# robustrobotics/multi_view_stereonet

Hardware: AMD Instinct MI355X
Metric: depthmaps/sec at 512x256, 64 hypotheses, 2 src views; L1 vs ref (higher is better)
Workload: dtype f32; 1 GPU; GTA-SfM-shaped 512x256, D=64 hypotheses, 2 source views, cost-volume filter + 5 refiners; global_batch=256, parallelism=dp1 (independent images, all-gather of metric rows)

## Files before the change

multi_view_stereonet_amd/csrc/mvsn_conv_wino.hip:

```cpp
#include <type_traits>
#include <utility>

#include "mvsn_resident.h"
#include "mvsn_conv_wino.h"

namespace mvsn {

constexpr int WN_THREADS = 512, WN_WAVES = 8;
constexpr int WN_TY = 16, WN_TX = 32;
constexpr int WN_WIDE_TY = 10, WN_WIDE_TX = 40, WN_WIDE_PC = WN_WIDE_TX / 2, WN_WIDE_NP = (WN_WIDE_TY / 2) * WN_WIDE_PC;
constexpr int WN_ROLL_PR = 6, WN_ROLL_NP = WN_ROLL_PR * WN_WIDE_PC, WN_ROLL_HY = 2 * WN_ROLL_PR + 3;
constexpr int WN_TILE_RP = 3;
constexpr int wn_pa(int dil) { return (dil + 3) / 4 * 4; }
constexpr int WN_UFLOATS = 16 * 128;
constexpr int WN_MAX_CHUNKS = 9;
constexpr int WN_LDS_MAX = 160 * 1024;

__device__ floatx4 g_wn_zero16 = {0.f, 0.f, 0.f, 0.f};

#ifndef MVSN_WN_ABLATE
#define MVSN_WN_ABLATE 0
#endif

#ifndef MVSN_RD_ABLATE
// ... 796 lines not shown
#pragma unroll
      for (int rr = 0; rr < 2; ++rr) {
        const bool rok = rr ? row1 : row0;
#pragma unroll
        for (int h = 0; h < 2; ++h) {
          const bool ok = rok && (h ? q1 : q0);
          if (rok && (!(MVSN_WN_ABLATE & 64) || n < 0))
            wn_store4<MVSN_WN_NT_STORES ? 2 : 0>(
                osrd, h ? ovoff1 : ovoff0, (unsigned)(((size_t)(t * 16) * cstride + (size_t)rr * DIL * g.W) * 4),
                floatx4{y[t][rr][4 * h], y[t][rr][4 * h + 1], y[t][rr][4 * h + 2], y[t][rr][4 * h + 3]});
          if (ok) {
#pragma unroll
            for (int k = 0; k < 4; ++k) s[t] += y[t][rr][4 * h + k];
          }
        }
      }
    }
    WN_STAMP();
    if (out_partials != nullptr) {
      auto sum8 = [](float v) {
        v += dpp_mov<0xB1>(v);
        v += dpp_mov<0x4E>(v);
        v += dpp_mov<0x141>(v);
        return v;
      };
      const int hi = (lq >> 3) & 1;
      const float npos = 8.0f * (float)cnt;
      const float rn = cnt == 16 ? 0.0078125f : (cnt == 8 ? 0.015625f : (cnt == 4 ? 0.03125f : 0.0f));
      float m[2], qv[2] = {0.f, 0.f};
#pragma unroll
      for (int t = 0; t < 2; ++t) {
        s[t] = sum8(s[t]);
        m[t] = s[t] * rn;
      }
#pragma unroll
      for (int t = 0; t < 2; ++t)
#pragma unroll
        for (int rr = 0; rr < 2; ++rr)
#pragma unroll
          for (int h = 0; h < 2; ++h)
            if ((rr ? row1 : row0) && (h ? q1 : q0)) {
#pragma unroll
              for (int k = 0; k < 4; ++k) {
                const float dv = y[t][rr][4 * h + k] - m[t];
                qv[t] += dv * dv;
              }
            }
#pragma unroll
      for (int t = 0; t < 2; ++t) qv[t] = sum8(qv[t]);
      int rtile = tile_id, rwave = wave;
      bool rec_ok = true;
      if constexpr (RP) {
        const int yq = oy & (TY - 1);
        rtile = (oy / TY) * g.ntx + x0 / TX, rwave = yq / (2 * DIL) * DIL + yq % DIL;
        rec_ok = oy < g.nty * TY;
      }
      if ((lq & 7) == 0 && rec_ok) {
        float *rec = out_partials + (((size_t)n * (RP ? g.tiles : ptiles) + (size_t)z * g.tiles + rtile) * WN_WAVES + rwave) * 48;
        rec += gq * 12 + hi * 3;
#pragma unroll
        for (int t = 0; t < 2; ++t) {
          rec[t * 6 + 0] = npos;
          rec[t * 6 + 1] = m[t];
          rec[t * 6 + 2] = qv[t];
        }
      }
    }
  };

  auto finish_tile_tr = [&](int n, int z, int tile_id, int y0, int x0, int r_s) {
    int lq;
    asm volatile("v_mbcnt_lo_u32_b32 %0, -1, 0\n\tv_mbcnt_hi_u32_b32 %0, -1, %0" : "=v"(lq));
    const int pc = lq & 15, gq = lq >> 4;
    int oy = y0 + 2 * wave, ox = x0 + 2 * pc;
    bool slot_ok = true;
    unsigned zb = 0;
    if constexpr (WIDE != 0) {
      const int q = wave * 16 + pc;
      slot_ok = q < NP;
      const int qq = slot_ok ? q : 0, pr = qq / WN_WIDE_PC;
      oy = y0 + 2 * pr, ox = x0 + 2 * (qq - pr * WN_WIDE_PC);
      if constexpr (ROLL) {
        const bool pb = pr >= r_s;
        oy = pb ? 2 * (pr - r_s) : oy;
        zb = pb ? (unsigned)plane : 0u;
        slot_ok = slot_ok & (!pb | (z + 1 < g.D));
      }
    }
    const bool row0 = oy < g.H, row1 = oy + 1 < g.H, cok = slot_ok && ox < g.W;
    const size_t cstride = VOL ? (size_t)g.D * plane : plane;
    const __amdgpu_buffer_rsrc_t osrd = wn_rsrc(out + (size_t)n * 32 * cstride + (size_t)z * plane, (unsigned)(32 * cstride * 4));
    const unsigned ovoff = cok ? ((unsigned)(4 * gq) * (unsigned)cstride + zb + (unsigned)(oy * g.W + ox)) * 4u : 0xFFFFFFFFu;
    const unsigned ovoff0 = (!WIDE || row0) ? ovoff : 0xFFFFFFFFu, ovoff1 = (!WIDE || row1) ? ovoff : 0xFFFFFFFFu;
    float s[2] = {0.f, 0.f};
    float y[2][4][4];
#pragma unroll
    for (int t = 0; t < 2; ++t) {
      const floatx4 bv = *reinterpret_cast<const floatx4 *>(bias_lds + t * 16 + 4 * gq);
#pragma unroll
      for (int r = 0; r < 4; ++r) {
        float s0[4], s1[4];
#pragma unroll
        for (int j = 0; j < 4; ++j) {
          s0[j] = acc[j][t][r] + acc[4 + j][t][r] + acc[8 + j][t][r];
          s1[j] = acc[4 + j][t][r] - acc[8 + j][t][r] - acc[12 + j][t][r];
        }
        y[t][r][0] = s0[0] + s0[1] + s0[2] + bv[r];
        y[t][r][1] = s0[1] - s0[2] - s0[3] + bv[r];
        y[t][r][2] = s1[0] + s1[1] + s1[2] + bv[r];
        y[t][r][3] = s1[1] - s1[2] - s1[3] + bv[r];
        if (!(MVSN_WN_ABLATE & 64) || n < 0) {
          const unsigned so = (unsigned)((size_t)(t * 16 + r) * cstride * 4);
          if (WIDE || row0) wn_store2<MVSN_WN_NT_TR ? 2 : 0>(osrd, ovoff0, so, y[t][r][0], y[t][r][1]);
          if (WIDE || row1) wn_store2<MVSN_WN_NT_TR ? 2 : 0>(osrd, ovoff1, so + (unsigned)g.W * 4u, y[t][r][2], y[t][r][3]);
        }
        if (row0 && cok) s[t] += y[t][r][0] + y[t][r][1];
        if (row1 && cok) s[t] += y[t][r][2] + y[t][r][3];
      }
    }
    WN_STAMP();
    if (out_partials != nullptr) {
      auto sum16 = [](float v) {
        v += dpp_mov<0xB1>(v);
        v += dpp_mov<0x4E>(v);
        v += dpp_mov<0x141>(v);
        v += dpp_mov<0x140>(v);
        return v;
      };
      const int vp = (g.W - x0) >> 1;
      float npos = (float)(8 * ((row0 ? 1 : 0) + (row1 ? 1 : 0)) * (vp > 16 ? 16 : vp));
      if constexpr (WIDE != 0)
        npos = sum16(cok ? (float)(8 * ((row0 ? 1 : 0) + (row1 ? 1 : 0))) : 0.0f);
      float m[2], qv[2] = {0.f, 0.f};
#pragma unroll
      for (int t = 0; t < 2; ++t) {
        s[t] = sum16(s[t]);
        m[t] = npos > 0.f ? s[t] / npos : 0.f;
      }
#pragma unroll
      for (int t = 0; t < 2; ++t)
#pragma unroll
        for (int r = 0; r < 4; ++r)
#pragma unroll
          for (int k = 0; k < 4; ++k)
            if ((k < 2 ? row0 : row1) && cok) {
              const float dv = y[t][r][k] - m[t];
              qv[t] += dv * dv;
            }
#pragma unroll
      for (int t = 0; t < 2; ++t) qv[t] = sum16(qv[t]);
      if (pc < 4) {
        float *rec = out_partials + (((size_t)n * ptiles + (ROLL ? (size_t)0 : (size_t)z * g.tiles) + tile_id) * WN_WAVES + wave) * 48;
        rec += gq * 12 + pc * 3;
        const int ga = gq >> 1;
        const bool a = pc == ga, b = pc == 2 + ga;
        rec[0] = (a || b) ? npos : 0.f;
        rec[1] = a ? m[0] : (b ? m[1] : 0.f);
        rec[2] = a ? qv[0] : (b ? qv[1] : 0.f);
      }
    }
  };

  int step = 0, mm_stage = 0;
  for (int round = 0; round < my_items; ++round) {
#ifdef MVSN_WN_STAMPS
    dbg_on = round >= 3 || my_items < 4;
#endif
    const int flat = g.rev ? total - 1 - (round * G + slot) : round * G + slot;
    const int n = flat / ptiles;
    int tile_id = flat - n * ptiles, z = 0;
    int r_pr0 = 0, r_s = WN_ROLL_PR;
    if constexpr (ROLL) {
      roll_item(tile_id, z, r_pr0, r_s);
    } else if constexpr (VOL) {
      z = tile_id / g.tiles;
      tile_id -= z * g.tiles;
    }
    const int tyi = ROLL ? 0 : wdiv(tile_id, g.fd_ntx), txi = ROLL ? 0 : tile_id - tyi * g.ntx;
    const int y0 = ROLL ? 2 * r_pr0 : item_y0(tyi), x0 = txi * TX;

#pragma unroll
    for (int xi = 0; xi < 16; ++xi) asm volatile("" : "=v"(acc[xi][0]), "=v"(acc[xi][1]));

    int chunk = 0;
    auto do_step = [&](auto firstc) {
      const bool has_next = step + 1 < total_steps;
      bool waited = false;
      if constexpr (RIDE > 0) {
        if constexpr (ASM_RIDE) {
          if (rd_young != PERV) asm volatile("s_waitcnt vmcnt(0)" ::: "memory");
          asm volatile("s_waitcnt vmcnt(%0)" ::"n"(PERV) : "memory");
        } else if (rd_young == PERV) asm volatile("s_waitcnt vmcnt(%0)" ::"n"(PERV) : "memory");
        else if (rd_young == PER) asm volatile("s_waitcnt vmcnt(%0)" ::"n"(PER) : "memory");
        else if (VOL && rd_young == 2) asm volatile("s_waitcnt vmcnt(2)" ::: "memory");
        else asm volatile("s_waitcnt vmcnt(0)" ::: "memory");
        rd_consume(lane);
        waited = true;
      }
      if (has_next) {
        const int rest = total_steps - (step + 2);
        if (!waited) wait_landed(rest < 0 ? 0 : (rest < NSTAGE - 2 ? rest : NSTAGE - 2));
        xf_apply();
        WN_STAMP();
        if (!(MVSN_WN_ABLATE & 8)) wn_barrier<LDS_BARRIER>();
        if (MVSN_WN_STAGGER > 0 && wave >= 4) __builtin_amdgcn_s_sleep(MVSN_WN_STAGGER);
        WN_STAMP();
        xf_prepare();
      }
      rd_issue(flat, chunk);
      float dn[KS][4][4];
      if (has_next && !(MVSN_WN_ABLATE & 32)) {
        if (MVSN_WN_XF == 1) tr_load(dn);
        else if (MVSN_WN_XF == 0) tr_load(dn, 0, 1);
      }
      auto multiply = [&](auto first, auto hc) {
        constexpr bool FIRST = decltype(first)::value;
        constexpr int h = decltype(hc)::value;
        const float *ub = U + (VOL ? mm_stage : chunk) * UST + h * WN_UFLOATS + lane;
        float fb[2][2];
        fb[0][0] = ub[0], fb[0][1] = ub[64];
        auto tcol = [&](int i, int j) {
          const float d0 = dn[h][0][dslot(j)], d1 = dn[h][1][dslot(j)], d2 = dn[h][2][dslot(j)], d3 = dn[h][3][dslot(j)];
          return i == 0 ? d0 - d2 : (i == 1 ? d1 + d2 : (i == 2 ? d2 - d1 : d1 - d3));
        };
        constexpr bool INTER = MVSN_WN_XF == 1 || (MVSN_WN_XF == 0 && h == 0);
        float tc[4], tn[4];
        if constexpr (INTER) {
#pragma unroll
          for (int j = 0; j < 4; ++j) tc[j] = tcol(0, j);
        } else {
          if (has_next && !(MVSN_WN_ABLATE & 32)) tr_load(dn, h, h + 1);
        }
#pragma unroll
        for (int xi = 0; xi < 16; ++xi) {
          const int cur = xi & 1, ti = xi >> 2, tj = xi & 3;
          if (INTER && ti < 3) tn[tj] = tcol(ti + 1, tj);
          if (xi + 1 < 16 && !(MVSN_WN_ABLATE & 2)) {
            fb[cur ^ 1][0] = ub[(xi + 1) * 128];
            fb[cur ^ 1][1] = ub[(xi + 1) * 128 + 64];
          }
          if constexpr (FIRST) {
            acc[xi][0] = TR ? mfma16x16x4(fb[cur][0], v[h][xi], floatx4{0.f, 0.f, 0.f, 0.f})
                            : mfma16x16x4(v[h][xi], fb[cur][0], floatx4{0.f, 0.f, 0.f, 0.f});
            acc[xi][1] = TR ? mfma16x16x4(fb[cur][1], v[h][xi], floatx4{0.f, 0.f, 0.f, 0.f})
                            : mfma16x16x4(v[h][xi], fb[cur][1], floatx4{0.f, 0.f, 0.f, 0.f});
          } else {
            acc[xi][0] = TR ? mfma16x16x4(fb[cur][0], v[h][xi], acc[xi][0]) : mfma16x16x4(v[h][xi], fb[cur][0], acc[xi][0]);
            acc[xi][1] = TR ? mfma16x16x4(fb[cur][1], v[h][xi], acc[xi][1]) : mfma16x16x4(v[h][xi], fb[cur][1], acc[xi][1]);
          }
          if (h == 0 && xi == 1 && has_next && !(MVSN_WN_ABLATE & 4)) {
            pf_issue();
            uq_issue();
          }
          if constexpr (INTER) {
            if (!(MVSN_WN_ABLATE & 1)) {
              v[h][xi] = tj == 0 ? tc[0] - tc[2] : (tj == 1 ? tc[1] + tc[2] : (tj == 2 ? tc[2] - tc[1] : tc[1] - tc[3]));
              if (MVSN_WN_PIN) asm volatile("" : "+v"(v[h][xi]));
            }
            if (tj == 3) {
#pragma unroll
              for (int k = 0; k < 4; ++k) tc[k] = tn[k];
            }
          }
          __builtin_amdgcn_sched_barrier(0);
        }
        if constexpr (!INTER) {
          if (!(MVSN_WN_ABLATE & 1)) {
            tr_finish(dn, v, h, h + 1);
#pragma unroll
            for (int xi = 0; xi < 16; ++xi)
              if (MVSN_WN_PIN) asm volatile("" : "+v"(v[h][xi]));
          }
          __builtin_amdgcn_sched_barrier(0);
        }
      };
      multiply(firstc, std::integral_constant<int, 0>{});
      if constexpr (KS == 2) multiply(std::false_type{}, std::integral_constant<int, 1>{});
      tr_advance();
      if constexpr (VOL) mm_stage = mm_stage + 1 == NSTAGE ? 0 : mm_stage + 1;
      WN_STAMP();
      ++step;
    };
    do_step(std::true_type{});
    for (chunk = 1; chunk < nsteps; ++chunk) do_step(std::false_type{});
    if (!(MVSN_WN_ABLATE & 16) || n < 0) {
      if constexpr (TR) finish_tile_tr(n, z, tile_id, y0, x0, r_s);
      else finish_tile(n, z, tile_id, y0, x0);
    }
  }
  if constexpr (RIDE > 0) {
    if (total_steps > 0) {
      asm volatile("s_waitcnt vmcnt(0)" ::: "memory");
      int ln;
      asm volatile("v_mbcnt_lo_u32_b32 %0, -1, 0\n\tv_mbcnt_hi_u32_b32 %0, -1, %0" : "=v"(ln));
      rd_consume(ln);
    }
  }
#ifdef MVSN_WN_STAMPS
  if (dbg)
    for (int i = 0; i < dbg_i; ++i) dbg[i] = dbg_lds[i];
#endif
}

constexpr int S2_TY = 16, S2_TX = 32;
constexpr int S2_ROWS = 2 * S2_TY + 3, S2_XS = 2 * S2_TX + 8, S2_DQ = S2_XS / 4;
constexpr int S2_GROUPS = S2_ROWS * S2_DQ, S2_PIECES = (S2_GROUPS + 63) / 64;
constexpr int S2_RCST = S2_ROWS * S2_XS + 1;
constexpr int S2_STAGE = 4 * S2_RCST;
constexpr int S2_UST = 4 * WN_UFLOATS;
constexpr int S2_STEPS = 8;
constexpr size_t S2_LDS_BYTES = (size_t)(2 * S2_STAGE + 2 * S2_UST + 32) * sizeof(float);
static_assert(S2_PIECES * 4 % WN_WAVES == 0, "a step's raw pieces divide evenly among the waves");
static_assert(S2_LDS_BYTES <= 160 * 1024, "LDS plan");

__global__ void wino_s2_pack_kernel(const float *__restrict__ w, float *__restrict__ out) {
  const int idx = blockIdx.x * blockDim.x + threadIdx.x;
  if (idx >= S2_STEPS * S2_UST) return;
  const int lane = idx & 63, t = (idx >> 6) & 1, xi = (idx >> 7) & 15, ph = (idx >> 11) & 3, cc = idx >> 13;
  const int py = ph >> 1, px = ph & 1;
  const int co = t * 16 + (lane & 15), ci = cc * 4 + (lane >> 4);
  const float *g = w + ((size_t)co * 32 + ci) * 25;
  const float G[4][3] = {{1.f, 0.f, 0.f}, {0.5f, 0.5f, 0.5f}, {0.5f, -0.5f, 0.5f}, {0.f, 0.f, 1.f}};
  const int i = xi >> 2, j = xi & 3;
  float u = 0.0f;
  for (int a = 0; a < 3; ++a)
    for (int b = 0; b < 3; ++b) {
      const int ky = 2 * a + py, kx = 2 * b + px;
      if (ky < 5 && kx < 5) u += G[i][a] * g[ky * 5 + kx] * G[j][b];
    }
  out[idx] = u;
}

#ifndef MVSN_S2_PIN
#define MVSN_S2_PIN 1
#endif
#ifndef MVSN_S2_CNTWAIT
#define MVSN_S2_CNTWAIT 1
#endif
struct WinoS2Args {
  int n, H, W, Ho, Wo, ntx, tiles;
  WinoDiv fd_ntx;
};

__global__ __launch_bounds__(WN_THREADS, 2) void conv_wino_s2_kernel(WinoS2Args g, const float *__restrict__ in,
                                                                     const float *__restrict__ upk,
                                                                     const float *__restrict__ bias,
                                                                     float *__restrict__ out) {
  extern __shared__ __attribute__((aligned(16))) float smem[];
  float *U = smem + 2 * S2_STAGE;
  float *bias_lds = U + 2 * S2_UST;
  const int tid = threadIdx.x, lane = tid & 63;
  const int wave = __builtin_amdgcn_readfirstlane(tid >> 6);
  const size_t plane = (size_t)g.H * g.W;
  const int oplane = g.Ho * g.Wo;
  const int total = g.n * g.tiles, G = gridDim.x;
  const int slot = xcd_tile_index(blockIdx.x, G);
  const int my_items = slot < total ? (total - slot + G - 1) / G : 0;
  const int total_steps = my_items * S2_STEPS;
  if (tid < 32) bias_lds[tid] = bias ? bias[tid] : 0.0f;

  constexpr int PER = S2_PIECES * 4 / WN_WAVES;
  const int dch = wave >> 1, dp0 = (wave & 1) * PER;
  int pf_item = 0, pf_cc = 0, pf_n = 0;
  int pf_goff[PER];
  auto pf_plan = [&]() {
    const int flat = pf_item * G + slot;
    const int n = flat / g.tiles, tile = flat - n * g.tiles;
    const int tyi = wdiv(tile, g.fd_ntx), txi = tile - tyi * g.ntx;
    const int gy0 = 2 * tyi * S2_TY - 2, gx0 = 2 * txi * S2_TX - 4;
    pf_n = n;
    int lo;
    asm volatile("v_mbcnt_lo_u32_b32 %0, -1, 0\n\tv_mbcnt_hi_u32_b32 %0, -1, %0" : "=v"(lo));
#pragma unroll
    for (int i = 0; i < PER; ++i) {
      const int e = (dp0 + i) * 64 + lo;
      const int row = e / S2_DQ, q = e - row * S2_DQ;
      const int gy = gy0 + row, gx = gx0 + 4 * q;
      pf_goff[i] = (gy >= 0 && gy < g.H && gx >= 0 && gx < g.W) ? (gy * g.W + gx) * 4 : -1;
    }
  };
  auto pf_issue = [&](int step) {
    if (step >= total_steps) return;
    const float *src = in + ((size_t)pf_n * 32 + pf_cc * 4 + dch) * plane;
    float *dst = smem + (step & 1) * S2_STAGE + dch * S2_RCST;
#pragma unroll
    for (int i = 0; i < PER; ++i)
      if ((dp0 + i) * 64 + lane < S2_GROUPS)
        wn_dma16_buf<true>(src, (unsigned)plane * 4u, (unsigned)pf_goff[i], dst + (dp0 + i) * 256);
    const float *us = upk + (size_t)pf_cc * S2_UST + wave * 1024 + lane * 4;
    float *ud = U + (step & 1) * S2_UST + wave * 1024;
#pragma unroll
    for (int i = 0; i < 4; ++i) wn_dma16<true>(us + i * 256, ud + i * 256);
    if (++pf_cc == S2_STEPS) {
      pf_cc = 0;
      ++pf_item;
      if (pf_item < my_items) pf_plan();
    }
  };
  if (my_items > 0) pf_plan();
  pf_issue(0);

  const int pcol = lane & 15, kc = lane >> 4;
  const int rbase = kc * S2_RCST + (4 * wave) * S2_XS + 4 * pcol + 2;

  floatx4 acc[16][2];
#pragma unroll
  for (int xi = 0; xi < 16; ++xi) acc[xi][0] = acc[xi][1] = floatx4{0.f, 0.f, 0.f, 0.f};

  int item = 0, cc = 0;
  for (int step = 0; step < total_steps; ++step) {
    if (MVSN_S2_CNTWAIT && cc == 0 && step > 0) asm volatile("s_waitcnt vmcnt(8)" ::: "memory");
    else asm volatile("s_waitcnt vmcnt(0)" ::: "memory");
    wn_barrier<true>();
    pf_issue(step + 1);
    const float *raw = smem + (step & 1) * S2_STAGE + rbase;
    const float *us = U + (step & 1) * S2_UST + lane;
#pragma unroll
    for (int py = 0; py < 2; ++py) {
      typedef float s2_f2 __attribute__((ext_vector_type(2)));
      s2_f2 d[4][4];
#pragma unroll
      for (int i = 0; i < 4; ++i)
#pragma unroll
        for (int j = 0; j < 4; ++j) {
          const float *q = raw + (py + 2 * i) * S2_XS + 2 * j;
          d[i][j] = (py && i == 3) ? s2_f2{0.f, 0.f} : s2_f2{q[0], q[1]};
        }
      s2_f2 t[4][4], v[16];
#pragma unroll
      for (int j = 0; j < 4; ++j) {
        t[0][j] = d[0][j] - d[2][j];
        t[1][j] = d[1][j] + d[2][j];
        t[2][j] = d[2][j] - d[1][j];
        t[3][j] = d[1][j] - d[3][j];
      }
#pragma unroll
      for (int i = 0; i < 4; ++i) {
        v[i * 4 + 0] = t[i][0] - t[i][2];
        v[i * 4 + 1] = t[i][1] + t[i][2];
        v[i * 4 + 2] = t[i][2] - t[i][1];
        v[i * 4 + 3] = t[i][1] - t[i][3];
      }
      if (MVSN_S2_PIN) {
#pragma unroll
        for (int xi = 0; xi < 16; ++xi)
          if (!(py && (xi >> 2) == 3)) asm volatile("" : "+v"(v[xi]));
      }
#pragma unroll
      for (int xi = 0; xi < 16; ++xi) {
        if (py && (xi >> 2) == 3) continue;
        const float *u = us + ((py * 2) * 16 + xi) * 128;
        acc[xi][0] = mfma16x16x4(v[xi].x, u[0], acc[xi][0]);
        acc[xi][1] = mfma16x16x4(v[xi].x, u[64], acc[xi][1]);
        if ((xi & 3) != 3) {
          acc[xi][0] = mfma16x16x4(v[xi].y, u[16 * 128], acc[xi][0]);
          acc[xi][1] = mfma16x16x4(v[xi].y, u[16 * 128 + 64], acc[xi][1]);
        }
      }
    }
    if (++cc == S2_STEPS) {
      cc = 0;
      const int flat = item * G + slot;
      const int n = flat / g.tiles, tile = flat - n * g.tiles;
      const int tyi = wdiv(tile, g.fd_ntx), txi = tile - tyi * g.ntx;
      const int y0 = tyi * S2_TY + 2 * wave, x0 = txi * S2_TX;
      const __amdgpu_buffer_rsrc_t osrd = wn_rsrc(out + (size_t)n * 32 * oplane, (unsigned)(32 * oplane) * 4u);
      int lo;
      asm volatile("v_mbcnt_lo_u32_b32 %0, -1, 0\n\tv_mbcnt_hi_u32_b32 %0, -1, %0" : "=v"(lo));
      const int ocl = lo & 15, oq = lo >> 4;
      unsigned ovoff[2];
#pragma unroll
      for (int hx = 0; hx < 2; ++hx)
        ovoff[hx] = x0 + 8 * oq + 4 * hx < g.Wo ? (unsigned)((ocl * oplane + 8 * oq + 4 * hx) * 4) : 0xFFFFFFFFu;
#pragma unroll
      for (int tt = 0; tt < 2; ++tt) {
        const float bv = bias_lds[tt * 16 + ocl];
        float y[4][2][2];
#pragma unroll
        for (int r = 0; r < 4; ++r) {
          float tm[2][4];
#pragma unroll
          for (int j = 0; j < 4; ++j) {
            tm[0][j] = acc[0 + j][tt][r] + acc[4 + j][tt][r] + acc[8 + j][tt][r];
            tm[1][j] = acc[4 + j][tt][r] - acc[8 + j][tt][r] - acc[12 + j][tt][r];
          }
#pragma unroll
          for (int a = 0; a < 2; ++a) {
            y[r][a][0] = tm[a][0] + tm[a][1] + tm[a][2] + bv;
            y[r][a][1] = tm[a][1] - tm[a][2] - tm[a][3] + bv;
          }
        }
#pragma unroll
        for (int a = 0; a < 2; ++a) {
          const bool rok = y0 + a < g.Ho;
          const unsigned so = rok ? (unsigned)((tt * 16 * oplane + (y0 + a) * g.Wo + x0) * 4) : 0u;
          wn_store4<0>(osrd, rok ? ovoff[0] : 0xFFFFFFFFu, so, floatx4{y[0][a][0], y[0][a][1], y[1][a][0], y[1][a][1]});
          wn_store4<0>(osrd, rok ? ovoff[1] : 0xFFFFFFFFu, so, floatx4{y[2][a][0], y[2][a][1], y[3][a][0], y[3][a][1]});
        }
      }
#pragma unroll
      for (int xi = 0; xi < 16; ++xi) acc[xi][0] = acc[xi][1] = floatx4{0.f, 0.f, 0.f, 0.f};
      ++item;
    }
  }
}

static int g_wn_rowphase = 0;

bool wino_geom(const mvsn_conv_desc *d, WinoGeom *g) {
  if (!d || d->precision != MVSN_CONV_FP32_WINO) return false;
  g->rpy = 0;
  if (d->n <= 0 || d->c_in <= 0 || d->c_out != 32 || d->depth < 1 || d->rows <= 0 || d->cols <= 0) return false;
  g->s2 = false;
  if (d->kd == 1 && d->kh == 5 && d->kw == 5 && d->stride == 2) {
    if (d->c_in != 32 || d->dilation != 1 || d->depth != 1 || d->cols % 8 != 0) return false;
    if ((unsigned long long)d->rows * d->cols * 32ull * 4ull >= (1ull << 31)) return false;
    g->s2 = true, g->wide = 0;
    g->n = d->n, g->cin = 32, g->H = d->rows, g->W = d->cols, g->dil = 1, g->D = 1, g->vol = false;
    g->nty = ((d->rows - 1) / 2 + 1 + S2_TY - 1) / S2_TY;
    g->ntx = ((d->cols - 1) / 2 + 1 + S2_TX - 1) / S2_TX;
    g->tiles = g->nty * g->ntx;
    g->nchunks = S2_STEPS * 4;
    g->packed_floats = (size_t)S2_STEPS * S2_UST;
    return (long)g->n * g->tiles < (1L << 30);
  }
  if ((d->kd != 1 && d->kd != 3) || d->kh != 3 || d->kw != 3 || d->stride != 1) return false;
  if (d->kd == 1 && d->depth != 1) return false;
  if (d->dilation != 1 && d->dilation != 2 && d->dilation != 4 && d->dilation != 8) return false;
  if (d->cols % 4 != 0) return false;
  if ((unsigned long long)d->depth * d->rows * d->cols * 32ull * 4ull >= (1ull << 32)) return false;
  g->n = d->n, g->cin = d->c_in, g->H = d->rows, g->W = d->cols, g->dil = d->dilation;
  g->D = d->depth, g->vol = d->kd == 3;
  g->nty = (d->rows + WN_TY - 1) / WN_TY;
  g->ntx = (d->cols + WN_TX - 1) / WN_TX;
  g->wide = 0;
#ifndef MVSN_WN_NO_WIDE
  if (d->kd == 3 && d->cols > WN_TX && d->cols <= WN_WIDE_TX) {
    const int strips = (d->rows + WN_WIDE_TY - 1) / WN_WIDE_TY;
    if (strips < g->nty * g->ntx) g->wide = 1, g->nty = strips, g->ntx = 1;
  }
#endif
  g->tiles = g->nty * g->ntx;
#ifndef MVSN_WN_NO_ROLL
  if (d->kd == 3 && d->cols > WN_TX && d->cols <= WN_WIDE_TX && d->c_in == 32 && d->dilation == 1) {
    const int pr = (d->rows + 1) / 2;
    const long items = ((long)d->depth * pr + WN_ROLL_PR - 1) / WN_ROLL_PR;
    if (pr >= WN_ROLL_PR && items < (long)d->depth * g->tiles && items < (1L << 24))
      g->wide = 2, g->nty = 1, g->ntx = 1, g->tiles = (int)items;
  }
#endif
  if (g->vol) {
    if (d->c_in != 32 || d->dilation != 1) return false;
    if ((long)wino_items(*g) > 1L << 24) return false;
    g->nchunks = 24;
    g->packed_floats = (size_t)g->nchunks * WN_UFLOATS;
    return true;
  }
  g->nchunks = (d->c_in + 3) / 4;
  if (g->nchunks > WN_MAX_CHUNKS) return false;
  if (g->nchunks > 8 && d->dilation > 2) return false;
  if (g->nchunks == 1 && d->dilation != 1) return false;
  g->packed_floats = (size_t)g->nchunks * WN_UFLOATS;
#ifndef MVSN_WN_NO_ROWPHASE
  if (d->dilation > 1 && g_wn_rowphase != 2) {
    const int rpy = ((d->rows + d->dilation - 1) / d->dilation + WN_TY - 1) / WN_TY;
    if (g_wn_rowphase == 1 || d->dilation * rpy <= g->nty) g->rpy = rpy;
  }
#endif
  return true;
}

int wino_pack_2d(const float *weight, int cin, float *packed, hipStream_t stream) {
  const int nchunks = (cin + 3) / 4, total = nchunks * WN_UFLOATS;
  hipLaunchKernelGGL(wino_pack_kernel, dim3((total + 255) / 256), dim3(256), 0, stream, weight, cin, 32, nchunks, 1,
                     packed);
  return check_launch("wino_pack_2d");
}

int wino_pack(const mvsn_conv_desc *d, const float *weight, float *packed, hipStream_t stream) {
  WinoGeom g;
  if (!wino_geom(d, &g)) return MVSN_E_BADARG;
  if (g.s2) {
    hipLaunchKernelGGL(wino_s2_pack_kernel, dim3((S2_STEPS * S2_UST + 255) / 256), dim3(256), 0, stream, weight, packed);
    return check_launch("mvsn_conv_pack_weights(winograd, 5x5 stride 2)");
  }
  const int total = g.nchunks * WN_UFLOATS;
  hipLaunchKernelGGL(wino_pack_kernel, dim3((total + 255) / 256), dim3(256), 0, stream, weight, g.cin, 32, g.nchunks,
                     g.vol ? 3 : 1, packed);
  return check_launch("mvsn_conv_pack_weights(winograd)");
}

static int wino_select(const WinoGeom &g, bool job) {
  if (g.s2) return -1;
  const bool head = g.nchunks == 1, rp = g.rpy > 0;
  WinoForm f = {};
  f.dil = g.dil, f.vol = g.vol, f.tile = rp ? WN_TILE_RP : g.wide;
  f.fullw = MVSN_WN_FULLW_OK && g.vol && !g.wide && g.ntx == 1 && g.W <= WN_TX;
  f.ks = (head || (rp ? job && g.dil == 8 : g.dil == 8 || (job && g.dil == 4))) ? 1 : 2;
  const bool four = !job && ((!g.vol && g.nchunks <= 8 && (rp ? g.dil <= 4 : g.dil == 1)) || g.wide == 2);
  f.nstage = head ? 6 : (four ? 4 : 3);
  f.ride = !job ? 0 : (g.vol ? 1 : (g.nchunks == 8 ? f.ks : 0));
  if (job && !f.ride) return -1;
  const int row = wn_find_form(f);
  return row >= 0 && g.nchunks <= WN_FORMS[row].chunks ? row : -1;
}

bool wino_can_carry(const WinoGeom &g, const mvsn_apply_job *job) {
  const int row = wino_select(g, true);
  if (row < 0 || !job || !job->x || !job->stats || !job->gamma || !job->beta || !job->out || job->n <= 0) return false;
  const int r = WN_FORMS[row].ride;
  if (job->spatial <= 0 || job->spatial % (256 * r) != 0) return false;
  if (job->r_stats && !(job->residual && job->r_gamma && job->r_beta)) return false;
  if ((((size_t)job->x | (size_t)job->out | (size_t)job->residual) & 15) != 0) return false;
  const long units = (long)job->n * 32 * (job->spatial / 256);
  if (g.vol && job->residual) return false;
  const long capacity = (long)g.n * wino_work_items(g) * WN_FORMS[row].nsteps(g.nchunks) * WN_WAVES * r;
  return units <= capacity && capacity < (1L << 31) && units < (1L << 30);
}

int wino_launch(const WinoGeom &g, const float *in, const float *upk, const float *bias, const float *in_stats,
                const float *in_gamma, const float *in_beta, float *out, float *out_partials, hipStream_t stream,
                const WinoBlocks *blocks, const mvsn_apply_job *job) {
  if (g.s2) {
    if (blocks || job || in_stats || out_partials) {
      set_error("mvsn_conv_forward(winograd, 5x5 stride 2): no input transform, statistics, channel blocks or carried job");
      return MVSN_E_BADARG;
    }
    WinoS2Args a;
    a.n = g.n, a.H = g.H, a.W = g.W, a.Ho = (g.H - 1) / 2 + 1, a.Wo = (g.W - 1) / 2 + 1, a.ntx = g.ntx, a.tiles = g.tiles;
    a.fd_ntx = wino_div((unsigned)g.ntx);
    static LdsOptIn opt;
    if (int rc = ensure_lds(opt, (const void *)conv_wino_s2_kernel, S2_LDS_BYTES, "mvsn_conv_forward(winograd, 5x5 stride 2)"))
      return rc;
    const long total = (long)g.n * g.tiles;
    const int cus = device_cus();
    hipLaunchKernelGGL(conv_wino_s2_kernel, dim3((unsigned)(total < cus ? total : cus)), dim3(WN_THREADS), S2_LDS_BYTES,
                       stream, a, in, upk, bias, out);
    return check_launch("mvsn_conv_forward(winograd, 5x5 stride 2)");
  }
  RideArgs rd = {};
  if (job) {
    if (blocks || !wino_can_carry(g, job)) {
      set_error("mvsn_conv_forward(winograd): this launch cannot carry the job");
      return MVSN_E_BADARG;
    }
    rd.x = job->x, rd.stats = job->stats, rd.gamma = job->gamma, rd.beta = job->beta;
    rd.res = job->residual, rd.r_stats = job->r_stats, rd.r_gamma = job->r_gamma, rd.r_beta = job->r_beta;
    rd.out = job->out;
    rd.units = (int)((long)job->n * 32 * (job->spatial / 256));
    rd.fd_upp = wino_div((unsigned)(job->spatial / 256));
  }
  WinoArgs a;
  a.n = g.n, a.cin = g.cin, a.H = g.H, a.W = g.W, a.ntx = g.ntx, a.tiles = g.tiles, a.nchunks = g.nchunks;
  a.fd_ntx = wino_div((unsigned)g.ntx);
  a.cb0 = g.cin, a.cb1 = 0, a.in1 = a.in2 = in;
  a.D = g.D;
  a.pr = (g.H + 1) / 2, a.fd_pr = wino_div((unsigned)a.pr);
  a.nty = g.nty, a.rpy = g.rpy;
  if (blocks) a.cb0 = blocks->cb0, a.cb1 = blocks->cb1, a.in1 = blocks->in1, a.in2 = blocks->in2;
  a.rev = (job && job->reverse == 1) ? 1 : 0;
  a.cs0 = (size_t)g.H * g.W, a.bs0 = (size_t)a.cb0 * a.cs0;
  if (blocks && blocks->cs0) a.cs0 = blocks->cs0, a.bs0 = blocks->bs0;
  const int row = wino_select(g, job != nullptr);
  if (row < 0) {
    set_error("mvsn_conv_forward(winograd): no kernel form for this layer");
    return MVSN_E_BADARG;
  }
  const size_t lds = WN_FORMS[row].bytes(g.nchunks);
  const int cus = device_cus();
  const long total = (long)g.n * wino_work_items(g);
  const dim3 grid((unsigned)(total < cus ? total : cus));
  auto launch = [&](auto mode, auto I) -> int {
    constexpr WinoForm F = WN_FORMS[decltype(I)::value];
    const auto kernel = conv_wino_kernel<decltype(mode)::value, F.ks, F.nstage, F.dil, F.vol, F.ride, F.tile, F.fullw>;
    static LdsOptIn opt;
    if (int rc = ensure_lds(opt, (const void *)kernel, lds, "mvsn_conv_forward(winograd)")) return rc;
    hipLaunchKernelGGL(kernel, grid, dim3(WN_THREADS), lds, stream, a, in, upk, bias, in_stats, in_gamma, in_beta, out,
                       out_partials, rd, (const void *)a.in1, (const void *)a.in2, (const void *)rd.x,
                       (const void *)rd.stats, (const void *)rd.res, (const void *)rd.r_stats, (const void *)rd.out,
                       (const void *)nullptr, (const void *)nullptr, (const void *)nullptr);
    return 0;
  };
  const bool xf = in_stats != nullptr;
  if (int rc = with_form_row(row, std::make_index_sequence<WN_NFORMS>{}, [&](auto I) {
        return xf ? launch(std::integral_constant<int, 1>{}, I) : launch(std::integral_constant<int, 0>{}, I);
      }))
    return rc;
  return check_launch("mvsn_conv_forward(winograd)");
}

}

extern "C" int mvsn_debug_set_wino_rowphase(int mode) {
  const int old = mvsn::g_wn_rowphase;
  mvsn::g_wn_rowphase = mode;
  return old;
}

extern "C" int mvsn_debug_wino_plan(const mvsn_conv_desc *desc, int carrying, int out[8]) {
  mvsn::WinoGeom g;
  if (!out || !mvsn::wino_geom(desc, &g)) return 0;
  const int row = mvsn::wino_select(g, carrying != 0);
  if (row < 0) return 0;
  const mvsn::WinoForm &f = mvsn::WN_FORMS[row];
  out[0] = f.ks, out[1] = f.nstage, out[2] = f.ride, out[3] = f.tile, out[4] = f.fullw;
  out[5] = (int)f.bytes(g.nchunks), out[6] = (int)mvsn::wino_work_items(g), out[7] = f.nsteps(g.nchunks);
  return 1;
}

#ifdef MVSN_WN_STAMPS
extern "C" int mvsn_debug_set_wino_stamps(void *buf) {
  return (int)hipMemcpyToSymbol(HIP_SYMBOL(mvsn::g_wn_stamps), &buf, sizeof(buf));
}
#endif
```

Measured before the change: 3921 depthmaps/s.

## Compact stride-2 Winograd weight blocks and spread prefetch DMA through the MFMA loop

```diff
diff --git a/multi_view_stereonet_amd/csrc/mvsn_conv_wino.hip b/multi_view_stereonet_amd/csrc/mvsn_conv_wino.hip
--- a/multi_view_stereonet_amd/csrc/mvsn_conv_wino.hip
+++ b/multi_view_stereonet_amd/csrc/mvsn_conv_wino.hip
@@ -1122,21 +1122,70 @@
 #endif
 }
 
+#ifndef MVSN_S2_FULL_U
+#define MVSN_S2_FULL_U 0
+#endif
+constexpr bool s2_live(int py, int px, int xi) { return !(py && (xi >> 2) == 3) && !(px && (xi & 3) == 3); }
+constexpr int s2_ublock(int py, int px, int xi) {
+  return MVSN_S2_FULL_U ? (py * 2 + px) * 16 + xi : py * 28 + 2 * xi - (xi >> 2) + px;
+}
+constexpr int S2_UBLOCKS = MVSN_S2_FULL_U ? 64 : 49;
+struct S2UTable {
+  int n;
+  int at[64];
+};
+constexpr S2UTable s2_utable() {
+  S2UTable t{};
+  for (int i = 0; i < 64; ++i) t.at[i] = -1;
+  for (int py = 0; py < 2; ++py)
+    for (int xi = 0; xi < 16; ++xi) {
+      if (py && (xi >> 2) == 3) continue;
+      for (int px = 0; px < 2; ++px) {
+        if (px && (xi & 3) == 3) continue;
+        t.at[(py * 2 + px) * 16 + xi] = MVSN_S2_FULL_U ? (py * 2 + px) * 16 + xi : t.n;
+        ++t.n;
+      }
+    }
+  return t;
+}
+constexpr S2UTable S2_UTABLE = s2_utable();
+constexpr bool s2_utable_ok() {
+  for (int f = 0; f < 64; ++f) {
+    const int py = f >> 5, px = (f >> 4) & 1, xi = f & 15;
+    if (s2_live(py, px, xi) != (S2_UTABLE.at[f] >= 0)) return false;
+    if (S2_UTABLE.at[f] >= 0 && (S2_UTABLE.at[f] != s2_ublock(py, px, xi) || S2_UTABLE.at[f] >= S2_UBLOCKS)) return false;
+  }
+  return true;
+}
+static_assert(S2_UTABLE.n == 49, "the multiply loop reads 49 of the 64 (phase, xi) blocks");
+static_assert(s2_utable_ok(), "s2_ublock disagrees with the multiply loop's skips");
 constexpr int S2_TY = 16, S2_TX = 32;
 constexpr int S2_ROWS = 2 * S2_TY + 3, S2_XS = 2 * S2_TX + 8, S2_DQ = S2_XS / 4;
 constexpr int S2_GROUPS = S2_ROWS * S2_DQ, S2_PIECES = (S2_GROUPS + 63) / 64;
 constexpr int S2_RCST = S2_ROWS * S2_XS + 1;
 constexpr int S2_STAGE = 4 * S2_RCST;
-constexpr int S2_UST = 4 * WN_UFLOATS;
+constexpr int S2_UST = S2_UBLOCKS * 128;
+constexpr int S2_UPIECES = (S2_UST + 255) / 256;
+constexpr int S2_UPER = S2_UPIECES / WN_WAVES;
 constexpr int S2_STEPS = 8;
-constexpr size_t S2_LDS_BYTES = (size_t)(2 * S2_STAGE + 2 * S2_UST + 32) * sizeof(float);
+#ifdef MVSN_S2_STAMPS
+constexpr int S2_STAMPS = 256;
+#else
+constexpr int S2_STAMPS = 0;
+#endif
+constexpr size_t S2_LDS_BYTES = (size_t)(2 * S2_STAGE + 2 * S2_UST + 32) * sizeof(float) + S2_STAMPS * 8;
 static_assert(S2_PIECES * 4 % WN_WAVES == 0, "a step's raw pieces divide evenly among the waves");
+static_assert(S2_UST % 4 == 0 && 2 * S2_STAGE % 4 == 0, "U stages start on 16 bytes (DMA pieces)");
 static_assert(S2_LDS_BYTES <= 160 * 1024, "LDS plan");
 
 __global__ void wino_s2_pack_kernel(const float *__restrict__ w, float *__restrict__ out) {
   const int idx = blockIdx.x * blockDim.x + threadIdx.x;
   if (idx >= S2_STEPS * S2_UST) return;
-  const int lane = idx & 63, t = (idx >> 6) & 1, xi = (idx >> 7) & 15, ph = (idx >> 11) & 3, cc = idx >> 13;
+  const int lane = idx & 63, t = (idx >> 6) & 1, cc = idx / S2_UST, blk = (idx - cc * S2_UST) >> 7;
+  int ph = 0, xi = 0;
+  for (int f = 0; f < 64; ++f)
+    if (s2_live(f >> 5, (f >> 4) & 1, f & 15) && s2_ublock(f >> 5, (f >> 4) & 1, f & 15) == blk) ph = f >> 4, xi = f & 15;
+  if (MVSN_S2_FULL_U) ph = blk >> 4, xi = blk & 15;
   const int py = ph >> 1, px = ph & 1;
   const int co = t * 16 + (lane & 15), ci = cc * 4 + (lane >> 4);
   const float *g = w + ((size_t)co * 32 + ci) * 25;
@@ -1157,10 +1206,19 @@
 #ifndef MVSN_S2_CNTWAIT
 #define MVSN_S2_CNTWAIT 1
 #endif
+#ifndef MVSN_S2_SPREAD
+#define MVSN_S2_SPREAD 1
+#endif
 struct WinoS2Args {
   int n, H, W, Ho, Wo, ntx, tiles;
   WinoDiv fd_ntx;
 };
+#ifdef MVSN_S2_STAMPS
+__device__ unsigned long long *g_s2_stamps = nullptr;
+#define S2_STAMP() do { if (dbg && dbg_on && dbg_i < S2_STAMPS) dbg_lds[dbg_i++] = __builtin_readcyclecounter(); } while (0)
+#else
+#define S2_STAMP() do { } while (0)
+#endif
 
 __global__ __launch_bounds__(WN_THREADS, 2) void conv_wino_s2_kernel(WinoS2Args g, const float *__restrict__ in,
                                                                      const float *__restrict__ upk,
@@ -1178,6 +1236,15 @@
   const int my_items = slot < total ? (total - slot + G - 1) / G : 0;
   const int total_steps = my_items * S2_STEPS;
   if (tid < 32) bias_lds[tid] = bias ? bias[tid] : 0.0f;
+#ifdef MVSN_S2_STAMPS
+#ifndef MVSN_S2_STAMP_WAVE
+#define MVSN_S2_STAMP_WAVE 0
+#endif
+  unsigned long long *dbg = (blockIdx.x == gridDim.x / 3 && tid == MVSN_S2_STAMP_WAVE * 64) ? g_s2_stamps : nullptr;
+  unsigned long long *dbg_lds = reinterpret_cast<unsigned long long *>(bias_lds + 32);
+  int dbg_i = 0;
+  bool dbg_on = false;
+#endif
 
   constexpr int PER = S2_PIECES * 4 / WN_WAVES;
   const int dch = wave >> 1, dp0 = (wave & 1) * PER;
@@ -1199,26 +1266,37 @@
       pf_goff[i] = (gy >= 0 && gy < g.H && gx >= 0 && gx < g.W) ? (gy * g.W + gx) * 4 : -1;
     }
   };
-  auto pf_issue = [&](int step) {
+  constexpr int S2_UTAIL = S2_UPIECES - S2_UPER * WN_WAVES;
+  constexpr int S2_NPF = PER + S2_UPER + (S2_UTAIL > 0 ? 1 : 0);
+  auto pf_piece = [&](int step, int k) {
     if (step >= total_steps) return;
-    const float *src = in + ((size_t)pf_n * 32 + pf_cc * 4 + dch) * plane;
-    float *dst = smem + (step & 1) * S2_STAGE + dch * S2_RCST;
-#pragma unroll
-    for (int i = 0; i < PER; ++i)
-      if ((dp0 + i) * 64 + lane < S2_GROUPS)
-        wn_dma16_buf<true>(src, (unsigned)plane * 4u, (unsigned)pf_goff[i], dst + (dp0 + i) * 256);
-    const float *us = upk + (size_t)pf_cc * S2_UST + wave * 1024 + lane * 4;
-    float *ud = U + (step & 1) * S2_UST + wave * 1024;
-#pragma unroll
-    for (int i = 0; i < 4; ++i) wn_dma16<true>(us + i * 256, ud + i * 256);
+    if (k < PER) {
+      const float *src = in + ((size_t)pf_n * 32 + pf_cc * 4 + dch) * plane;
+      float *dst = smem + (step & 1) * S2_STAGE + dch * S2_RCST;
+      if ((dp0 + k) * 64 + lane < S2_GROUPS)
+        wn_dma16_buf<true>(src, (unsigned)plane * 4u, (unsigned)pf_goff[k], dst + (dp0 + k) * 256);
+    } else if (k < PER + S2_UPER) {
+      const int p = wave * S2_UPER + (k - PER);
+      wn_dma16<true>(upk + (size_t)pf_cc * S2_UST + p * 256 + lane * 4, U + (step & 1) * S2_UST + p * 256);
+    } else if (wave < S2_UTAIL) {
+      const int p = S2_UPER * WN_WAVES + wave;
+      if (p * 256 + lane * 4 < S2_UST)
+        wn_dma16<true>(upk + (size_t)pf_cc * S2_UST + p * 256 + lane * 4, U + (step & 1) * S2_UST + p * 256);
+    }
+  };
+  auto pf_next = [&](int step) {
+    if (step >= total_steps) return;
     if (++pf_cc == S2_STEPS) {
       pf_cc = 0;
       ++pf_item;
       if (pf_item < my_items) pf_plan();
     }
   };
+  static_assert(S2_NPF <= 16, "one piece per xi of the even row phase");
   if (my_items > 0) pf_plan();
-  pf_issue(0);
+#pragma unroll
+  for (int k = 0; k < S2_NPF; ++k) pf_piece(0, k);
+  pf_next(0);
 
   const int pcol = lane & 15, kc = lane >> 4;
   const int rbase = kc * S2_RCST + (4 * wave) * S2_XS + 4 * pcol + 2;
@@ -1229,10 +1307,26 @@
 
   int item = 0, cc = 0;
   for (int step = 0; step < total_steps; ++step) {
+#ifdef MVSN_S2_STAMPS
+    if (cc == 0) {
+      const bool on = item >= 3 || my_items < 4;
+      if (on && !dbg_on) {
+        dbg_on = true;
+        S2_STAMP();
+      }
+    }
+#endif
     if (MVSN_S2_CNTWAIT && cc == 0 && step > 0) asm volatile("s_waitcnt vmcnt(8)" ::: "memory");
     else asm volatile("s_waitcnt vmcnt(0)" ::: "memory");
+    S2_STAMP();
     wn_barrier<true>();
-    pf_issue(step + 1);
+    S2_STAMP();
+    if (!MVSN_S2_SPREAD) {
+#pragma unroll
+      for (int k = 0; k < S2_NPF; ++k) pf_piece(step + 1, k);
+      pf_next(step + 1);
+    }
+    S2_STAMP();
     const float *raw = smem + (step & 1) * S2_STAGE + rbase;
     const float *us = U + (step & 1) * S2_UST + lane;
 #pragma unroll
@@ -1269,14 +1363,20 @@
 #pragma unroll
       for (int xi = 0; xi < 16; ++xi) {
         if (py && (xi >> 2) == 3) continue;
-        const float *u = us + ((py * 2) * 16 + xi) * 128;
+        if (MVSN_S2_SPREAD && py == 0 && xi < S2_NPF) {
+          pf_piece(step + 1, xi);
+          if (xi == S2_NPF - 1) pf_next(step + 1);
+        }
+        const float *u = us + s2_ublock(py, 0, xi) * 128;
         acc[xi][0] = mfma16x16x4(v[xi].x, u[0], acc[xi][0]);
         acc[xi][1] = mfma16x16x4(v[xi].x, u[64], acc[xi][1]);
         if ((xi & 3) != 3) {
-          acc[xi][0] = mfma16x16x4(v[xi].y, u[16 * 128], acc[xi][0]);
-          acc[xi][1] = mfma16x16x4(v[xi].y, u[16 * 128 + 64], acc[xi][1]);
-        }
-      }
+          const float *u1 = us + s2_ublock(py, 1, xi) * 128;
+          acc[xi][0] = mfma16x16x4(v[xi].y, u1[0], acc[xi][0]);
+          acc[xi][1] = mfma16x16x4(v[xi].y, u1[64], acc[xi][1]);
+        }
+      }
+      S2_STAMP();
     }
     if (++cc == S2_STEPS) {
       cc = 0;
@@ -1321,8 +1421,13 @@
 #pragma unroll
       for (int xi = 0; xi < 16; ++xi) acc[xi][0] = acc[xi][1] = floatx4{0.f, 0.f, 0.f, 0.f};
       ++item;
-    }
-  }
+      S2_STAMP();
+    }
+  }
+#ifdef MVSN_S2_STAMPS
+  if (dbg)
+    for (int i = 0; i < dbg_i; ++i) dbg[i] = dbg_lds[i];
+#endif
 }
 
 static int g_wn_rowphase = 0;
@@ -1533,3 +1638,8 @@
   return (int)hipMemcpyToSymbol(HIP_SYMBOL(mvsn::g_wn_stamps), &buf, sizeof(buf));
 }
 #endif
+#ifdef MVSN_S2_STAMPS
+extern "C" int mvsn_debug_set_s2_stamps(void *buf) {
+  return (int)hipMemcpyToSymbol(HIP_SYMBOL(mvsn::g_s2_stamps), &buf, sizeof(buf));
+}
+#endif
```

Result: no change. 3920 depthmaps/s, median of 2 (-0.0%).
